# apple/ml-stable-diffusion

Hardware: AMD Instinct MI355X
Metric: diffusion iter/s (UNet steps/s), SD2.1-base 512x512 fp16 (higher is better)
Workload: dtype fp16; 1 GPU; BASELINE config 2: SD2.1-base (865.9 M-parameter UNet), random-init, denoising iteration at 512x512 (64x64 latents), CFG batch 2 per prompt, DDIM, device-resident loop; unet=sd21-base, latent=64, attention=ORIGINAL, prompts_per_gpu=1, global_batch=2, hip_graph=True, parallelism=dp1 (independent prompts per rank, no data-path collective)

## Files before the change

### include/sd_mi355x.h

```cpp
#ifndef SD_MI355X_H
#define SD_MI355X_H

#include <stddef.h>
#include <stdint.h>

#ifdef __cplusplus
extern "C" {
#endif

typedef enum sd_status {
  SD_OK = 0,
  SD_ERR_INVALID_ARGUMENT = -1,
  SD_ERR_NOT_FOUND = -2,
  SD_ERR_HIP = -3,
  SD_ERR_UNSUPPORTED = -4,
  SD_ERR_INTERNAL = -5
} sd_status;

typedef enum sd_dtype { SD_F16 = 0, SD_F32 = 1 } sd_dtype;

typedef enum sd_attention_impl {
  SD_ATTN_ORIGINAL = 0,
  SD_ATTN_SPLIT_EINSUM = 1,
  SD_ATTN_SPLIT_EINSUM_V2 = 2
// ... 103 lines not shown
int sd_text_encoder_encode(sd_text_encoder* t, const int32_t* input_ids, int eos_index, float* last_hidden_state,
                           float* hidden_embeds, float* pooled);

int sd_op_attention(int impl, const void* q, const void* k, const void* v, void* out, int B, int heads, int d,
                    int Sq, int Sk, int variant, int iters, float* ms);
int sd_op_layernorm(const void* x, const float* weight, const float* bias, void* out, int B, int C, int S, float eps,
                    int iters, float* ms);
int sd_op_groupnorm(const void* x, const float* weight, const float* bias, void* out, int B, int C, int H, int W,
                    int groups, float eps, int silu, int iters, float* ms);
int sd_op_groupnorm_shortcut(const void* x0, const void* x1, const float* gn_weight, const float* gn_bias, const void* w, const float* bias,
                             void* out_gn, void* out_sc, int B, int C0, int C1, int H, int W, int N, int groups, float eps, int silu,
                             int side, int iters, float* ms);
int sd_op_conv2d(const void* x, const void* w, const float* bias, const void* res, void* out, int B, int Cin, int H,
                 int W, int Cout, int ksize, int stride, int upsample, int tile, int splitk, int force_generic,
                 int iters, float* ms);
int sd_op_conv2d_groupnorm(const void* x, const void* w, const float* bias, const void* res, const float* gn_weight,
                           const float* gn_bias, void* conv_out, void* out, int B, int Cin, int H, int W, int Cout, int ksize,
                           int groups, float eps, int silu, int tile, int producer_stats, int* entries, int iters, float* ms);
int sd_op_conv2d_groupnorm_proj(const void* x, const void* w, const float* bias, const void* res, const float* gn_weight,
                                const float* gn_bias, const void* proj_w, const float* proj_bias, void* conv_out, void* out, int B,
                                int Cin, int H, int W, int Cout, int ksize, int Nproj, int groups, float eps, int fold, int tile,
                                int* entries, int iters, float* ms);
int sd_op_conv2d_groupnorm_conv3x3(const void* x, const void* w, const float* bias, const void* res, const float* gn_weight,
                                   const float* gn_bias, const void* w2, const float* bias2, const void* res2, void* conv_out, void* out,
                                   int B, int Cin, int H, int W, int Cout, int ksize, int N2, int groups, float eps, int silu, int fold,
                                   int tile, int staging2, int* entries, int iters, float* ms);
int sd_op_ffn_out_proj(const void* g, const void* w1, const float* b1, const void* res1, const void* w2, const float* b2, const void* res2,
                       void* out, float* gn_sums, int B, int C, int S, int groups, int fused, int iters, float* ms);
int sd_op_cross_attention_fused(const void* x, const float* ln_weight, const float* ln_bias, const void* wq, const void* k,
                                const void* v, void* out, int B, int heads, int Sq, int Sk, float eps, int nst, int iters,
// ... 25 lines not shown
```

### ml-stable-diffusion_amd/csrc/capi.cpp

```cpp
#include <cmath>
#include <cstdlib>
#include <cstring>

#include "unet.h"

namespace sd {
extern thread_local std::string g_last_error;
int selftest_mfma();

namespace {

template <typename F>
int guarded(F&& f) {
  try {
    f();
    g_last_error.clear();
    return kOk;
  } catch (const Error& e) {
    g_last_error = e.what();
    return e.code;
  } catch (const std::bad_alloc&) {
    g_last_error = "out of host memory";
    return kInternal;
  } catch (const std::exception& e) {
// ... 452 lines not shown
    const size_t on = (size_t)B * Ho * Wo * Cout;
    half_t* dout = sc.dev<half_t>(on);
    d.out = dout;
    d.B = B; d.Hi = H; d.Wi = W; d.Ho = Ho; d.Wo = Wo;
    d.ksize = ksize; d.stride = stride; d.up = up; d.N = Cout;
    d.tile = tile % 10;
    d.staging = tile / 10;
    if (tile >= 110 && tile <= 116) {
      d.tile = 11;
      d.staging = tile - 110;
    }
    if (tile >= 140 && tile <= 142) {
      d.tile = 12;
      d.staging = tile - 140;
    }
    d.splitk = splitk;
    d.debug = force_generic >= 2 ? force_generic - 1 : 0;
    if (d.debug & 4) d.prof = sc.dev<long long>(8);
    const bool fast = force_generic != 1 && conv_fast_path_ok(d);
    ConvWorkspace ws;
    if (fast && d.tile == 9) {
      SD_REQUIRE(wstream_shape_ok(d), kInvalidArgument, "conv2d: shape not eligible for plan tile 9 (wstream.hip)");
      half_t* wtd = sc.dev<half_t>(wstream_tiled_halves(Cout, Cin, ksize));
      launch_wstream_retile(d.w, wtd, Cout, Cin, ksize, sc.stream);
      d.w_tiled = wtd;
    }
    if (fast && d.tile == 11) {
      SD_REQUIRE(bvgemm_shape_ok(d), kInvalidArgument, "conv2d: shape not eligible for plan tile 11 (bvgemm.hip)");
      half_t* wtd = sc.dev<half_t>(bvgemm_tiled_halves(Cout, Cin));
      launch_bvgemm_retile(d.w, wtd, Cout, Cin, false, sc.stream);
// ... 9 lines not shown
        launch_conv(d, ws, sc.stream);
      else if (small_n)
        launch_conv_small_n(d, nullptr, sc.stream);
      else
        launch_conv_generic(d, 0, sc.stream);
    });
    if (d.prof) {
      long long t[8];
      SD_HIP(hipMemcpy(t, d.prof, sizeof(t), hipMemcpyDeviceToHost));
      fprintf(stderr, "[sd prof] block0: prologue %lld, k-loop %lld, epilogue %lld shader cycles; total %lld cycles = %lld ticks of the 100 MHz wall clock\n",
              t[1] - t[0], t[2] - t[1], t[3] - t[2], t[3] - t[0], t[4]);
    }
    std::vector<half_t> ot(on);
    SD_HIP(hipMemcpy(ot.data(), dout, on * 2, hipMemcpyDeviceToHost));
    nhwc_to_nchw(ot.data(), reinterpret_cast<half_t*>(out), B, Cout, Ho, Wo);
  });
}

int sd_op_conv2d_groupnorm(const void* x, const void* w, const float* bias, const void* res, const float* gn_weight,
                           const float* gn_bias, void* conv_out, void* out, int B, int Cin, int H, int W, int Cout, int ksize,
                           int groups, float eps, int silu, int tile, int producer_stats, int* entries, int iters, float* ms) {
  return guarded([&] {
    SD_REQUIRE(x && w && gn_weight && gn_bias && out, kInvalidArgument, "NULL argument");
    SD_REQUIRE(ksize == 1 || ksize == 3, kInvalidArgument, "conv2d_groupnorm: ksize %d", ksize);
    Scratch sc;
    std::vector<half_t> xt = nchw_to_nhwc(reinterpret_cast<const half_t*>(x), B, Cin, H, W);
    const half_t* wh = reinterpret_cast<const half_t*>(w);
    const int kk = ksize * ksize;
    std::vector<half_t> wt((size_t)Cout * Cin * kk);
    for (int o = 0; o < Cout; ++o)
// ... 5 lines not shown
    d.w = sc.dev<half_t>(wt.size(), wt.data());
    d.bias = bias ? sc.dev<float>(Cout, bias) : nullptr;
    std::vector<half_t> rt;
    if (res) {
      rt = nchw_to_nhwc(reinterpret_cast<const half_t*>(res), B, Cout, H, W);
      d.res = sc.dev<half_t>(rt.size(), rt.data());
    }
    const size_t on = (size_t)B * H * W * Cout;
    half_t* dconv = sc.dev<half_t>(on);
    half_t* dy = sc.dev<half_t>(on);
    d.out = dconv;
    d.B = B; d.Hi = H; d.Wi = W; d.Ho = H; d.Wo = W;
    d.ksize = ksize; d.stride = 1; d.up = 1; d.N = Cout;
    d.tile = tile % 10;
    d.staging = tile / 10;
    d.splitk = 1;
    const bool fast = conv_fast_path_ok(d);
    float* partial = sc.dev<float>(groupnorm_scratch_floats(B, H * W, groups));
    {
      std::vector<float> poison(groupnorm_scratch_floats(B, H * W, groups), 1.0e30f);
      SD_HIP(hipMemcpy(partial, poison.data(), poison.size() * sizeof(float), hipMemcpyHostToDevice));
    }
    if (producer_stats == 1) {
      d.gn_partial = partial;
      d.gn_groups = groups;
    }
    float* dgw = sc.dev<float>(Cout, gn_weight);
    float* dgb = sc.dev<float>(Cout, gn_bias);
    ConvWorkspace ws;
    if (fast && d.tile == 9) {
// ... 937 lines not shown
```

### ml-stable-diffusion_amd/csrc/igemm.hip

```cpp
#include <cstdio>
#include <cstdlib>
#include <cstring>
#include <string>
#include <type_traits>

#include "kernels.h"

namespace sd {

namespace {

constexpr int BK = 64;
constexpr int LDS_ROW = BK + 8;

struct IgemmArgs {
  const half_t* x0;
  const half_t* x1;
  const half_t* w;
  const float* bias;
  const float* temb;
  const half_t* res;
  half_t* out;
  float* partial;
  int C0, C1, Ctot;
// ... 91 lines not shown

__device__ __forceinline__ float xor32_sum(float v) {
  const unsigned u = __float_as_uint(v);
  const auto r = __builtin_amdgcn_permlane32_swap(u, u, false, false);
  const unsigned r0 = r[0], r1 = r[1];
  return __uint_as_float(r0) + __uint_as_float(r1);
}

__device__ __forceinline__ float wave_sum(float v) {
#pragma unroll
  for (int o = 32; o > 0; o >>= 1) v += __shfl_xor(v, o);
  return v;
}
#include "gn_body.inc"

__device__ __forceinline__ void dma16_to_lds(const __amdgpu_buffer_rsrc_t& rs, char* lds, unsigned voffset, int soffset) {
#if defined(__HIP_DEVICE_COMPILE__)
  __builtin_amdgcn_raw_ptr_buffer_load_lds(rs, (__attribute__((address_space(3))) void*)lds, 16, voffset, soffset, 0, 0);
#endif
}

template <int BM, int BN, int WGM, int WGN, int TM, int TN, bool LNF, int NRES = 0>
__device__ __forceinline__ void tile_epilogue(const IgemmArgs& a, floatx16 (&acc)[TM][TN], const float (&ln_a)[TM],
                                              const float (&ln_b)[TM], char* smem, float* sconst, float const_b, float const_t,
                                              float const_c, int m_blk, int n_blk, int wave, int split, bool temb_uniform,
                                              const half8* resv = nullptr, bool use_resv = false) {
  const int tid = threadIdx.x, lane = tid & 63;
  const int wm = wave / WGN, wn = wave % WGN;
  const int frow = lane & 31, hi = lane >> 5;
  if (a.slab) {
#pragma unroll
    for (int i = 0; i < TM; ++i) {
      const int m = m_blk + (wm * TM + i) * 32 + frow;
      if (m >= a.M) continue;
      float* prow = a.partial + ((size_t)split * a.M + m) * a.N;
// ... 579 lines not shown
    tile_epilogue<BM, BN, WGM, WGN, TM, TN, LNF, (RES_PRE ? RIT : 0)>(a, acc, ln_a, ln_b, smem, sconst, const_b, const_t, const_c, m_blk,
                                                                      n_blk, wave, split, temb_uniform, resv, use_resv);
  }
  if (prof) {
    prof_t[3] = clock64();
    a.prof[0] = prof_t[0];
    a.prof[1] = prof_t[1];
    a.prof[2] = prof_t[2];
    a.prof[3] = prof_t[3];
    a.prof[4] = wall_clock64() - prof_w0;
  }
}

constexpr int HALO_W = 18, HALO_ROWS = 180, HALO_PIECES = 23, HALO_LDS_ROWS = 184, HALO_PPW = 6;

template <int N>
__device__ __forceinline__ void wait_vmcnt_barrier() {
  asm volatile("s_waitcnt vmcnt(%0)\n\ts_barrier" ::"n"(N) : "memory");
}
constexpr int halo_mod9(int t) { return ((t % 9) + 9) % 9; }
template <bool GNL = false>
constexpr int halo_x_issued(int tap) {
  const int t = halo_mod9(tap);
  return GNL ? (t == 0 ? 2 : (t <= 4 ? 1 : 0)) : (t < HALO_PPW ? 1 : 0);
}
constexpr size_t halo_lds_bytes(int bn, int d) {
  return ((size_t)2 * HALO_LDS_ROWS * BK + (size_t)d * bn * BK) * sizeof(half_t) + bn * sizeof(float);
}

template <int D, int WR, bool GNL = false>
constexpr int halo_ks_wait_count(int tap) {
  int n = 0;
  for (int i = 2; i <= D - 1; ++i) n += WR + halo_x_issued<GNL>(tap - D + i);
  if (tap == 8 && n > 2 * WR) n = 2 * WR;
// ... 1736 lines not shown
    }
  }
  if (d.tile == 11) {
    SD_REQUIRE(d.w_bv && bvgemm_shape_ok(d), kInvalidArgument, "plan tile 11 (bvgemm.hip) needs the pre-tiled weights and an eligible 1x1 shape");
    launch_bvgemm(d, d.staging, s);
    return 0;
  }
  {
    static const bool sm_on = tune_env_int("SD_SMGEMM", 1) != 0;
    const bool forced = d.tile == 12;
    if (forced || (sm_on && d.tile == 0 && d.splitk == 0 && d.staging == 0 && g_tune.tile == 0 && smgemm_wanted(d))) {
      launch_smgemm(d, forced ? d.staging : 0, s);
      return 0;
    }
  }
  IgemmArgs a = make_args(d);
  Plan p = choose_plan(d, a);
  bool halo = p.tile == 7;
  const bool twins = d.n_twins > 0;
  SD_REQUIRE(!twins || (d.out_mode == kOutHalf && !d.ln_colsum && !d.out_t && !d.debug && reduce_twin_ok(a.HoWo, a.N, d.n_twins, d.twin)),
             kInvalidArgument, "GroupNorm twins need a plain fp16 output and whole (sample, group) slices (HoWo=%d N=%d)", a.HoWo, a.N);
  if (d.gnf_partial && d.ksize == 3) {
    SD_REQUIRE(conv_gn_loader_ok(d) && d.gnf_silu == 1 && d.gnf_gamma && d.gnf_beta && d.gnf_entries >= 1 && d.gnf_entries <= 128 && !twins, kInvalidArgument,
               "GroupNorm in the conv loader: Ctot=%d groups=%d entries=%d up=%d", a.Ctot, d.gnf_groups, d.gnf_entries, d.up);
    p.tile = 7;
    if (p.staging != 2 && p.staging != 3) p.staging = 3;
    p.splitk = 1;
  } else if (d.gnf_partial) {
    SD_REQUIRE(d.ksize == 1 && d.stride == 1 && !d.x1 && d.out_mode == kOutHalf && !d.ln_colsum && !d.out_t && !twins && gemm_pipe_ok(a) &&
                   d.gnf_gamma && d.gnf_beta && d.gnf_groups >= 1 && d.gnf_groups <= 32 && a.K % d.gnf_groups == 0 && a.K <= 2048 &&
// ... 185 lines not shown
```

### ml-stable-diffusion_amd/csrc/kernels.h

```cpp
#pragma once
#include "sd_common.h"

namespace sd {

enum OutMode : int {
  kOutHalf = 0,
  kOutHalfT = 1,
  kOutGeglu = 2,
};

struct GnTwin {
  half_t* y = nullptr;
  int ld = 0, c_off = 0;
  int cpg = 0;
  const float* gamma = nullptr;
  const float* beta = nullptr;
  float eps = 1e-5f;
  int silu = 0;
};

struct ConvDesc {
  const half_t* x0 = nullptr;
  const half_t* x1 = nullptr;
  int C0 = 0, C1 = 0;
// ... 65 lines not shown
bool wsgemm_wanted(const ConvDesc& d);
size_t wsgemm_tiled_halves(int N);
void launch_wsgemm_retile(const half_t* w, half_t* wt, int N, bool geglu, hipStream_t s);
void launch_wsgemm(const ConvDesc& d, hipStream_t s);

bool bvgemm_shape_ok(const ConvDesc& d);
size_t bvgemm_tiled_halves(int N, int K);
void launch_bvgemm_retile(const half_t* w, half_t* wt, int N, int K, bool geglu, hipStream_t s);
void launch_bvgemm(const ConvDesc& d, int variant, hipStream_t s);
bool bvgemm_wanted(const ConvDesc& d);

bool smgemm_shape_ok(const ConvDesc& d, int variant);
bool smgemm_wanted(const ConvDesc& d);
void launch_smgemm(const ConvDesc& d, int variant, hipStream_t s);

void run_calibration(int device, float* out);

int launch_conv_generic(const ConvDesc& d, int act_silu_out, hipStream_t s);

void launch_conv_small_n(const ConvDesc& d, float* out_nchw_f32, hipStream_t s);

enum AttnImpl : int { kAttnOriginal = 0, kAttnSplitEinsum = 1, kAttnSplitEinsumV2 = 2 };

struct AttnDesc {
  const half_t* q = nullptr;
  const half_t* k = nullptr;
  const half_t* vt = nullptr;
  half_t* out = nullptr;
  int B = 1, heads = 1, d = 64, Sq = 0, Sk = 0;
  int ldq = 0, ldk = 0, ldv = 0, ldo = 0;
// ... 165 lines not shown
```

### ml-stable-diffusion_amd/csrc/sd_common.h

```cpp
#pragma once
#include <hip/hip_runtime.h>

#include <cstdint>
#include <cstdio>
#include <cstdlib>
#include <map>
#include <memory>
#include <stdexcept>
#include <string>
#include <atomic>
#include <vector>

namespace sd {

typedef _Float16 half_t;
typedef _Float16 half8 __attribute__((ext_vector_type(8)));
typedef _Float16 half4 __attribute__((ext_vector_type(4)));
typedef _Float16 half2v __attribute__((ext_vector_type(2)));
typedef float floatx16 __attribute__((ext_vector_type(16)));
typedef float floatx4 __attribute__((ext_vector_type(4)));

template <typename V>
__device__ __forceinline__ void out_store(V* p, const V& v) {
#if defined(SD_SC1_STORES) && defined(__HIP_DEVICE_COMPILE__)
  if constexpr (sizeof(V) == 16) {
    typedef unsigned u4_ __attribute__((ext_vector_type(4)));
    asm volatile("global_store_dwordx4 %0, %1, off sc1\n\ts_nop 1" ::"v"(p), "v"(__builtin_bit_cast(u4_, v)) : "memory");
  } else if constexpr (sizeof(V) == 8) {
    typedef unsigned u2_ __attribute__((ext_vector_type(2)));
    asm volatile("global_store_dwordx2 %0, %1, off sc1\n\ts_nop 1" ::"v"(p), "v"(__builtin_bit_cast(u2_, v)) : "memory");
  } else {
    *p = v;
  }
#else
  *p = v;
#endif
}

enum Status : int {
  kOk = 0,
  kInvalidArgument = -1,
  kNotFound = -2,
  kHipError = -3,
  kUnsupported = -4,
  kInternal = -5,
};

struct Error : std::runtime_error {
  int code;
  Error(int c, const std::string& m) : std::runtime_error(m), code(c) {}
};
// ... 75 lines not shown
```

### ml-stable-diffusion_amd/python_hip_stable_diffusion/_lib.py

```python
import ctypes as C
import os

import numpy as np

_HERE = os.path.dirname(os.path.abspath(__file__))
LIB_PATH = os.environ.get("SD_MI355X_LIB", os.path.join(os.path.dirname(_HERE), "lib", "libsdmi355.so"))

SD_MAX_LEVELS = 6
SD_FLAG_DEVICE_PTRS = 1
ATTENTION_IMPLEMENTATIONS = {"ORIGINAL": 0, "SPLIT_EINSUM": 1, "SPLIT_EINSUM_V2": 2}


class LibraryNotBuilt(ImportError):
    pass


class UNetConfig(C.Structure):
    _fields_ = [
        ("batch", C.c_int32), ("in_channels", C.c_int32), ("out_channels", C.c_int32),
        ("height", C.c_int32), ("width", C.c_int32), ("n_levels", C.c_int32),
        ("block_out_channels", C.c_int32 * SD_MAX_LEVELS),
        ("down_cross_attn", C.c_int32 * SD_MAX_LEVELS),
        ("up_cross_attn", C.c_int32 * SD_MAX_LEVELS),
        ("layers_per_block", C.c_int32),
# ... 46 lines not shown
    ("sd_unet_attach_controlnets", _I, [_P, C.POINTER(_P), _I]),
    ("sd_controlnet_set_cond", _I, [_P, _P, _I]),
    ("sd_vae_decoder_create", _I, [C.POINTER(UNetConfig), _P, _I, C.POINTER(_P)]),
    ("sd_vae_decode", _I, [_P, _P, _I, _FP, _I]),
    ("sd_vae_encoder_create", _I, [C.POINTER(UNetConfig), _P, _I, C.POINTER(_P)]),
    ("sd_vae_encode", _I, [_P, _P, _I, _FP, _I]),
    ("sd_text_encoder_create", _I, [_P, _P, _I, C.POINTER(_P)]),
    ("sd_text_encoder_destroy", None, [_P]),
    ("sd_text_encoder_device_bytes", C.c_size_t, [_P]),
    ("sd_text_encoder_encode", _I, [_P, C.POINTER(C.c_int32), _I, _FP, _FP, _FP]),
    ("sd_op_attention", _I, [_I, _P, _P, _P, _P, _I, _I, _I, _I, _I, _I, _I, _FP]),
    ("sd_op_layernorm", _I, [_P, _FP, _FP, _P, _I, _I, _I, _F, _I, _FP]),
    ("sd_op_groupnorm", _I, [_P, _FP, _FP, _P, _I, _I, _I, _I, _I, _F, _I, _I, _FP]),
    ("sd_op_groupnorm_shortcut", _I, [_P, _P, _FP, _FP, _P, _FP, _P, _P, _I, _I, _I, _I, _I, _I, _I, _F, _I, _I, _I, _FP]),
    ("sd_op_conv2d", _I, [_P, _P, _FP, _P, _P, _I, _I, _I, _I, _I, _I, _I, _I, _I, _I, _I, _I, _FP]),
    ("sd_op_conv2d_groupnorm", _I, [_P, _P, _FP, _P, _FP, _FP, _P, _P, _I, _I, _I, _I, _I, _I, _I, _F, _I, _I, _I, C.POINTER(_I), _I, _FP]),
    ("sd_op_conv2d_groupnorm_proj", _I, [_P, _P, _FP, _P, _FP, _FP, _P, _FP, _P, _P, _I, _I, _I, _I, _I, _I, _I, _I, _F, _I, _I, C.POINTER(_I), _I, _FP]),
    ("sd_op_conv2d_groupnorm_conv3x3", _I, [_P, _P, _FP, _P, _FP, _FP, _P, _FP, _P, _P, _P, _I, _I, _I, _I, _I, _I, _I, _I, _F, _I, _I, _I, _I,
                                            C.POINTER(_I), _I, _FP]),
    ("sd_op_cross_attention_fused", _I, [_P, _FP, _FP, _P, _P, _P, _P, _I, _I, _I, _I, _F, _I, _I, _FP]),
    ("sd_op_ffn_out_proj", _I, [_P, _P, _FP, _P, _P, _FP, _P, _P, _FP, _I, _I, _I, _I, _I, _I, _FP]),
    ("sd_op_cross_attention_block", _I, [_P, _FP, _FP, _P, _P, _P, _P, _FP, _P, _P, _FP, _P, _I, _I, _I, _I, _F, _I, _I, _FP]),
    ("sd_op_geglu", _I, [_P, _P, _FP, _P, _I, _I, _I, _I, _FP]),
    ("sd_op_geglu_ln", _I, [_P, _FP, _FP, _P, _FP, _P, _I, _I, _I, C.c_float, _I, _I, _FP]),
    ("sd_op_qkv_ln", _I, [_P, _FP, _FP, _P, _P, _P, _I, _I, _I, C.c_float, C.c_float, _I, _I, _I, _FP]),
    ("sd_op_gn_proj_qkv", _I, [_P, _P, _FP, _FP, _P, _FP, _FP, _FP, _P, _P, _P, _P, _I, _I, _I, _I, _I, C.c_float, C.c_float, C.c_float, _I, _I,
                               C.POINTER(C.c_int), _I, _FP]),
    ("sd_op_timestep_embedding", _I, [_FP, _FP, _I, _I, _I, _F]),
    ("sd_numpy_randn", _I, [C.c_uint32, C.POINTER(C.c_double), C.c_size_t]),
    ("sd_torch_randn", _I, [C.c_uint32, C.POINTER(C.c_double), C.c_size_t]),
# ... 91 lines not shown
    if Cin2 != Cin or k != k2:
        raise ValueError("conv2d: weight shape does not match input")
    up = 2 if upsample else 1
    pad = k // 2
    Ho = (H * up + 2 * pad - k) // stride + 1
    Wo = (W * up + 2 * pad - k) // stride + 1
    bias = None if bias is None else f32(bias)
    res = None if res is None else f16(res)
    out = np.empty((B, Cout, Ho, Wo), np.float16)
    ms = C.c_float(0)
    check(lib().sd_op_conv2d(ptr(x), ptr(w), fptr(bias), ptr(res), ptr(out), B, Cin, H, W, Cout, k, stride,
                             int(upsample), tile, splitk, int(force_generic), iters, C.byref(ms)))
    return out, ms.value


def groupnorm_shortcut(x0, x1, gn_weight, gn_bias, w, bias=None, groups=32, eps=1e-5, silu=True, side=True, iters=1):
    x0, w = f16(x0), f16(w)
    x1 = None if x1 is None else f16(x1)
    B, C0, H, W = x0.shape
    C1 = 0 if x1 is None else x1.shape[1]
    N = w.shape[0]
    w = np.ascontiguousarray(w.reshape(N, -1))
    if w.shape[1] != C0 + C1 or (x1 is not None and x1.shape != (B, C1, H, W)):
        raise ValueError("groupnorm_shortcut: inconsistent shapes")
    gn_weight, gn_bias = f32(gn_weight), f32(gn_bias)
    bias = None if bias is None else f32(bias)
    out_gn = np.empty((B, C0 + C1, H, W), np.float16)
    out_sc = np.empty((B, N, H, W), np.float16)
    ms = C.c_float(0)
    check(lib().sd_op_groupnorm_shortcut(ptr(x0), ptr(x1), fptr(gn_weight), fptr(gn_bias), ptr(w), fptr(bias), ptr(out_gn), ptr(out_sc),
# ... 197 lines not shown
```

Baseline: 236.8 it/s.

## Add conv80 implicit-GEMM 3x3 conv kernel with BN=80 tiles and weight ring

Adds a new 3x3 stride-1 implicit-GEMM conv kernel that uses an 80-wide output-channel tile, a halo-staged activation tile and a D-deep ring of weight stages loaded via buffer-to-LDS DMA. It supports a concatenated second input, upsample-by-2, and bias, temb and residual epilogues. It is auto-selected when the tile count falls between 192 and 256, which aims to fill the CUs better for UNet channel counts such as 320, 640 and 1280 that are multiples of 80. It also adds a conv2d_cat test entry point. The cost is significant new kernel complexity and a risk of mis-selection on some shapes.

```diff
diff --git a/include/sd_mi355x.h b/include/sd_mi355x.h
--- a/include/sd_mi355x.h
+++ b/include/sd_mi355x.h
@@ -141,6 +141,8 @@
 int sd_op_conv2d(const void* x, const void* w, const float* bias, const void* res, void* out, int B, int Cin, int H,
                  int W, int Cout, int ksize, int stride, int upsample, int tile, int splitk, int force_generic,
                  int iters, float* ms);
+int sd_op_conv2d_cat(const void* x0, const void* x1, const void* w, const float* bias, const void* res, void* out, int B, int C0, int C1,
+                     int H, int W, int Cout, int tile, int iters, float* ms);
 int sd_op_conv2d_groupnorm(const void* x, const void* w, const float* bias, const void* res, const float* gn_weight,
                            const float* gn_bias, void* conv_out, void* out, int B, int Cin, int H, int W, int Cout, int ksize,
                            int groups, float eps, int silu, int tile, int producer_stats, int* entries, int iters, float* ms);
diff --git a/ml-stable-diffusion_amd/csrc/capi.cpp b/ml-stable-diffusion_amd/csrc/capi.cpp
--- a/ml-stable-diffusion_amd/csrc/capi.cpp
+++ b/ml-stable-diffusion_amd/csrc/capi.cpp
@@ -490,6 +490,10 @@
       d.tile = 12;
       d.staging = tile - 140;
     }
+    if (tile >= 150 && tile <= 152) {
+      d.tile = 13;
+      d.staging = tile - 150;
+    }
     d.splitk = splitk;
     d.debug = force_generic >= 2 ? force_generic - 1 : 0;
     if (d.debug & 4) d.prof = sc.dev<long long>(8);
@@ -529,6 +533,54 @@
     std::vector<half_t> ot(on);
     SD_HIP(hipMemcpy(ot.data(), dout, on * 2, hipMemcpyDeviceToHost));
     nhwc_to_nchw(ot.data(), reinterpret_cast<half_t*>(out), B, Cout, Ho, Wo);
+  });
+}
+
+int sd_op_conv2d_cat(const void* x0, const void* x1, const void* w, const float* bias, const void* res, void* out, int B, int C0, int C1,
+                     int H, int W, int Cout, int tile, int iters, float* ms) {
+  return guarded([&] {
+    SD_REQUIRE(x0 && x1 && w && out, kInvalidArgument, "NULL argument");
+    SD_REQUIRE(C0 > 0 && C1 > 0, kInvalidArgument, "conv2d_cat: C0 %d C1 %d", C0, C1);
+    Scratch sc;
+    const int Cin = C0 + C1;
+    std::vector<half_t> x0t = nchw_to_nhwc(reinterpret_cast<const half_t*>(x0), B, C0, H, W);
+    std::vector<half_t> x1t = nchw_to_nhwc(reinterpret_cast<const half_t*>(x1), B, C1, H, W);
+    const half_t* wh = reinterpret_cast<const half_t*>(w);
+    std::vector<half_t> wt((size_t)Cout * Cin * 9);
+    for (int o = 0; o < Cout; ++o)
+      for (int c = 0; c < Cin; ++c)
+        for (int t = 0; t < 9; ++t) wt[((size_t)o * 9 + t) * Cin + c] = wh[((size_t)o * Cin + c) * 9 + t];
+    ConvDesc d;
+    d.x0 = sc.dev<half_t>(x0t.size(), x0t.data());
+    d.C0 = C0;
+    d.x1 = sc.dev<half_t>(x1t.size(), x1t.data());
+    d.C1 = C1;
+    d.w = sc.dev<half_t>(wt.size(), wt.data());
+    d.bias = bias ? sc.dev<float>(Cout, bias) : nullptr;
+    std::vector<half_t> rt;
+    if (res) {
+      rt = nchw_to_nhwc(reinterpret_cast<const half_t*>(res), B, Cout, H, W);
+      d.res = sc.dev<half_t>(rt.size(), rt.data());
+    }
+    const size_t on = (size_t)B * H * W * Cout;
+    half_t* dout = sc.dev<half_t>(on);
+    d.out = dout;
+    d.B = B; d.Hi = H; d.Wi = W; d.Ho = H; d.Wo = W;
+    d.ksize = 3; d.stride = 1; d.up = 1; d.N = Cout;
+    d.tile = tile % 10;
+    d.staging = tile / 10;
+    if (tile >= 150 && tile <= 152) {
+      d.tile = 13;
+      d.staging = tile - 150;
+    }
+    SD_REQUIRE(conv_fast_path_ok(d), kInvalidArgument, "conv2d_cat: C0=%d C1=%d N=%d not MFMA-tileable", C0, C1, Cout);
+    ConvWorkspace ws;
+    ws.partial_bytes = conv_workspace_bytes(d);
+    if (ws.partial_bytes) ws.partial = reinterpret_cast<float*>(sc.dev<char>(ws.partial_bytes));
+    sc.timed(iters, ms, [&] { launch_conv(d, ws, sc.stream); });
+    std::vector<half_t> ot(on);
+    SD_HIP(hipMemcpy(ot.data(), dout, on * 2, hipMemcpyDeviceToHost));
+    nhwc_to_nchw(ot.data(), reinterpret_cast<half_t*>(out), B, Cout, H, W);
   });
 }
 
@@ -564,6 +616,10 @@
     d.ksize = ksize; d.stride = 1; d.up = 1; d.N = Cout;
     d.tile = tile % 10;
     d.staging = tile / 10;
+    if (tile >= 150 && tile <= 152) {
+      d.tile = 13;
+      d.staging = tile - 150;
+    }
     d.splitk = 1;
     const bool fast = conv_fast_path_ok(d);
     float* partial = sc.dev<float>(groupnorm_scratch_floats(B, H * W, groups));
diff --git a/ml-stable-diffusion_amd/csrc/conv80.hip b/ml-stable-diffusion_amd/csrc/conv80.hip
--- /dev/null
+++ b/ml-stable-diffusion_amd/csrc/conv80.hip
@@ -0,0 +1,519 @@
+#include <algorithm>
+#include <type_traits>
+
+#include "kernels.h"
+
+namespace sd {
+
+namespace {
+
+constexpr int C8_BK = 64;
+constexpr int C8_BN = 80;
+constexpr int C8_ROWB = 128;
+constexpr int C8_WR = 3;
+constexpr int C8_TN = C8_BN / 16;
+constexpr int C8_WSTAGE = C8_BN * C8_ROWB;
+
+struct C80Args {
+  const half_t* x0;
+  const half_t* x1;
+  const half_t* w;
+  const float* bias;
+  const float* temb;
+  const half_t* res;
+  half_t* out;
+  int C0, C1, Ctot;
+  int B, Hi, Wi, Ho, Wo, up;
+  int N, K;
+  int temb_stride, res_ld;
+  int has_bias, has_temb, has_res;
+  int tiles_x, tiles_y, n_fast;
+  float* gn_partial;
+  int gn_G, gn_cpg;
+};
+
+template <int BM>
+struct C80Geo {
+  static constexpr int TW = BM == 128 ? 16 : 8, TH = 8;
+  static constexpr int HW = TW + 2;
+  static constexpr int HROWS = (TH + 2) * HW;
+  static constexpr int PIECES = (HROWS + 7) / 8;
+  static constexpr int LDS_ROWS = PIECES * 8;
+  static constexpr int PPW = (PIECES + 3) / 4;
+  static constexpr int KY = BM == 128 ? 0 : 4;
+  static constexpr int TMB = BM / 32;
+  static constexpr int KEEP = TMB / 2;
+  static constexpr int HALO_B = LDS_ROWS * C8_ROWB;
+  static_assert(BM == 128 || BM == 64, "tile");
+  static_assert(PPW <= 8, "halo pieces go out in tap steps 0-7");
+};
+
+template <int BM>
+constexpr size_t c80_lds_bytes(int d) {
+  return (size_t)2 * C80Geo<BM>::HALO_B + (size_t)d * C8_WSTAGE + C8_BN * sizeof(float);
+}
+template <int BM>
+constexpr size_t c80_red_bytes() { return (size_t)4 * C80Geo<BM>::KEEP * C8_TN * 64 * 16; }
+constexpr int C8_OROW = C8_BN + 8;
+constexpr int C8_GN_RG = 16;
+
+constexpr int c80_mod9(int t) { return ((t % 9) + 9) % 9; }
+template <int D, int PPW, int MODE>
+constexpr int c80_wait_count(int tap) {
+  int n = 0;
+  for (int u = tap - D + 2; u <= tap - 1; ++u) {
+    if (MODE == 2) n += (u < 0 || u + D < 9) ? C8_WR : 0;
+    else n += C8_WR + ((MODE == 1 ? (u >= 0 && u < PPW) : (c80_mod9(u) < PPW)) ? 1 : 0);
+  }
+  if (MODE != 2 && tap == 8 && n > (8 - PPW) * C8_WR) n = (8 - PPW) * C8_WR;
+  return n;
+}
+template <int D, int PPW, int MODE>
+__device__ __forceinline__ void c80_wait(int tap) {
+  switch (tap) {
+    case 0: wait_vmcnt_barrier<c80_wait_count<D, PPW, MODE>(0)>(); break;
+    case 1: wait_vmcnt_barrier<c80_wait_count<D, PPW, MODE>(1)>(); break;
+    case 2: wait_vmcnt_barrier<c80_wait_count<D, PPW, MODE>(2)>(); break;
+    case 3: wait_vmcnt_barrier<c80_wait_count<D, PPW, MODE>(3)>(); break;
+    case 4: wait_vmcnt_barrier<c80_wait_count<D, PPW, MODE>(4)>(); break;
+    case 5: wait_vmcnt_barrier<c80_wait_count<D, PPW, MODE>(5)>(); break;
+    case 6: wait_vmcnt_barrier<c80_wait_count<D, PPW, MODE>(6)>(); break;
+    case 7: wait_vmcnt_barrier<c80_wait_count<D, PPW, MODE>(7)>(); break;
+    default: wait_vmcnt_barrier<c80_wait_count<D, PPW, MODE>(8)>(); break;
+  }
+}
+
+template <int BM, int D>
+__global__ __launch_bounds__(256, 1) void conv80_kernel(C80Args a) {
+  using G = C80Geo<BM>;
+  constexpr int TW = G::TW, HW = G::HW, PPW = G::PPW, TMB = G::TMB, KEEP = G::KEEP, KY = G::KY;
+  constexpr int ROWB = C8_ROWB, WR = C8_WR, TN = C8_TN, BK = C8_BK;
+  static_assert(D >= 3 && D <= 10, "ring depth: a step's tile is at most one chunk ahead of the chunk after it");
+  static_assert((D - 1) * (WR + 1) <= 63, "vmcnt range");
+  static_assert(c80_lds_bytes<BM>(D) <= 160 * 1024, "LDS");
+  static_assert(c80_red_bytes<BM>() + (size_t)BM * C8_OROW * 2 <= (size_t)2 * G::HALO_B + (size_t)D * C8_WSTAGE, "epilogue buffers fit the K-loop buffers");
+  static_assert((size_t)(C8_GN_RG * 10 * 17 + 2 * C8_BN) * 4 <= c80_red_bytes<BM>(), "statistics scratch fits the exchange buffer");
+  extern __shared__ __attribute__((aligned(16))) char smem[];
+  char* const Xh = smem;
+  char* const Ws = smem + 2 * G::HALO_B;
+  float* const sconst = reinterpret_cast<float*>(Ws + D * C8_WSTAGE);
+
+  const int tid = threadIdx.x, lane = tid & 63;
+  const int wave = __builtin_amdgcn_readfirstlane(tid >> 6);
+  const int wm = wave >> 1, wk = wave & 1;
+  const int g = lane >> 4, r16 = lane & 15;
+  const int H = a.Ho, W = a.Wo;
+  const int ush = a.up >> 1;
+
+  const int n_tiles = a.N / C8_BN;
+  const int m_tiles = a.B * a.tiles_y * a.tiles_x;
+  const int nwg = m_tiles * n_tiles;
+  int bid = blockIdx.x;
+  {
+    int q = nwg >> 3, r = nwg & 7, xcd = bid & 7, idx = bid >> 3;
+    int base = (xcd < r) ? xcd * (q + 1) : r * (q + 1) + (xcd - r) * q;
+    bid = base + idx;
+  }
+  const int bn_idx = a.n_fast ? bid % n_tiles : bid / m_tiles, mt = a.n_fast ? bid / n_tiles : bid % m_tiles;
+  const int b = mt / (a.tiles_y * a.tiles_x);
+  const int trem = mt - b * (a.tiles_y * a.tiles_x);
+  const int ty = trem / a.tiles_x, tx = trem - ty * a.tiles_x;
+  const int y0 = ty * G::TH, x0 = tx * TW;
+  const int n_blk = bn_idx * C8_BN;
+  const int nch = a.Ctot / BK;
+
+  constexpr int VW = KEEP == 2 ? 8 : 4;
+  typedef _Float16 ovec __attribute__((ext_vector_type(VW)));
+  const int opl = wm * (BM / 2) + 16 * (wk * KEEP + (KEEP == 2 ? (g & 1) : 0)) + r16;
+  const int oy = y0 + opl / TW, ox = x0 + opl % TW;
+  const bool o_ok = oy < H && ox < W;
+  const size_t om = (size_t)(b * H + min(oy, H - 1)) * W + min(ox, W - 1);
+  const int ocol = n_blk + (KEEP == 2 ? 8 * (g >> 1) : 4 * g);
+  ovec resv[TN];
+#pragma unroll
+  for (int j = 0; j < TN; ++j) resv[j] = *reinterpret_cast<const ovec*>(a.res + om * a.res_ld + ocol + 16 * j);
+  const int cn = n_blk + min(tid, C8_BN - 1);
+  const float const_b = a.bias[cn], const_t = a.temb[(size_t)b * a.temb_stride + cn];
+  __builtin_amdgcn_sched_barrier(0);
+
+  constexpr unsigned kOob = 0x80000000u;
+  const __amdgpu_buffer_rsrc_t rs_w = __builtin_amdgcn_make_buffer_rsrc(const_cast<half_t*>(a.w), 0, (int)((size_t)a.N * a.K * 2), 0x00020000);
+  const size_t xpix = (size_t)a.B * a.Hi * a.Wi;
+  auto piece_of = [&](int j) { return (wave + 4 * j < G::PIECES) ? wave + 4 * j : G::PIECES - 1; };
+  unsigned hoff0[PPW], hoff1[PPW];
+#pragma unroll
+  for (int j = 0; j < PPW; ++j) {
+    const int hr = 8 * piece_of(j) + (lane >> 3);
+    const int hy = hr / HW, hx = hr - hy * HW;
+    const int iy = y0 - 1 + hy, ix = x0 - 1 + hx;
+    const bool ok = (hr < G::HROWS) && iy >= 0 && iy < H && ix >= 0 && ix < W;
+    const unsigned pix = (unsigned)((b * a.Hi + (iy >> ush)) * a.Wi + (ix >> ush));
+    const unsigned sw = (unsigned)(((lane & 7) ^ (((hx >> 1) + KY * (hy & 1)) & 7)) * 16);
+    hoff0[j] = ok ? pix * (unsigned)a.C0 * 2u + sw : kOob;
+    hoff1[j] = ok ? pix * (unsigned)a.C1 * 2u + sw : kOob;
+  }
+  auto wpiece_of = [&](int i) { return (wave + 4 * i < C8_BN / 8) ? wave + 4 * i : wave + 4 * (i - 1); };
+  unsigned woff[WR];
+#pragma unroll
+  for (int i = 0; i < WR; ++i) {
+    const int r = 8 * wpiece_of(i) + (lane >> 3);
+    woff[i] = (unsigned)(n_blk + r) * (unsigned)a.K * 2u + (unsigned)(((lane & 7) ^ ((r >> 1) & 7)) * 16);
+  }
+#define HALO_SRC(rs, off, soff, ch)                                                                                        \
+  const bool rs##_second = (ch) * BK >= a.C0;                                                           \
+  const __amdgpu_buffer_rsrc_t rs = __builtin_amdgcn_make_buffer_rsrc(                                                     \
+      const_cast<half_t*>(rs##_second ? a.x1 : a.x0), 0, (int)(xpix * (rs##_second ? a.C1 : a.C0) * 2), 0x00020000);       \
+  const int soff = (rs##_second ? (ch) * BK - a.C0 : (ch) * BK) * 2;                                                       \
+  unsigned off[PPW];                                                                                                       \
+  _Pragma("unroll") for (int j_ = 0; j_ < PPW; ++j_) off[j_] = rs##_second ? hoff1[j_] : hoff0[j_];
+  auto issue_x_piece = [&](int j, const __amdgpu_buffer_rsrc_t& rs, unsigned off, int soff, int xstage) {
+    char* dst = Xh + xstage * G::HALO_B + piece_of(j) * 1024;
+    dma16_to_lds(rs, dst, off, soff);
+  };
+  const int total_steps = nch * 9;
+  int iw_koff = 0, iw_tap = 0, iw_slot = 0;
+  auto issue_next_w = [&]() {
+    char* ws = Ws + iw_slot * C8_WSTAGE;
+#pragma unroll
+    for (int i = 0; i < WR; ++i) dma16_to_lds(rs_w, ws + wpiece_of(i) * 1024, woff[i], iw_koff);
+    if (++iw_slot == D) iw_slot = 0;
+    iw_koff += a.Ctot * 2;
+    if (++iw_tap == 9) {
+      iw_tap = 0;
+      iw_koff += (BK - 9 * a.Ctot) * 2;
+    }
+  };
+
+  floatx4 acc[TMB][TN];
+#pragma unroll
+  for (int i = 0; i < TMB; ++i)
+#pragma unroll
+    for (int j = 0; j < TN; ++j) acc[i][j] = floatx4{0.f, 0.f, 0.f, 0.f};
+
+  const int kc = 4 * wk + g;
+  int hrb[TMB];
+  int fpy0 = 0, fpx = 0;
+#pragma unroll
+  for (int i = 0; i < TMB; ++i) {
+    const int ml = wm * (BM / 2) + 16 * i + r16;
+    const int py = ml / TW, px = ml % TW;
+    hrb[i] = (py * HW + px) * ROWB;
+    if (i == 0) { fpy0 = py; fpx = px; }
+  }
+  int xsw[KY ? 2 : 1][3];
+#pragma unroll
+  for (int p = 0; p < (KY ? 2 : 1); ++p)
+#pragma unroll
+    for (int kx = 0; kx < 3; ++kx) xsw[p][kx] = (kc ^ ((((fpx + kx) >> 1) + KY * ((fpy0 + p) & 1)) & 7)) * 16;
+  const int wsw = r16 * ROWB + (kc ^ ((r16 >> 1) & 7)) * 16;
+
+  auto read_step = [&](half8 (&xf)[TMB], half8 (&wf)[TN], const char* xs, const char* ws, int tap) {
+    const int ky = tap / 3, kx = tap - ky * 3;
+    const int toffb = (ky * HW + kx) * ROWB;
+#pragma unroll
+    for (int i = 0; i < TMB; ++i) xf[i] = *reinterpret_cast<const half8*>(xs + hrb[i] + toffb + xsw[KY ? (ky & 1) : 0][kx]);
+#pragma unroll
+    for (int j = 0; j < TN; ++j) wf[j] = *reinterpret_cast<const half8*>(ws + j * 16 * ROWB + wsw);
+  };
+  auto mfma_step = [&](half8 (&xf)[TMB], half8 (&wf)[TN]) {
+#pragma unroll
+    for (int i = 0; i < TMB; ++i)
+#pragma unroll
+      for (int j = 0; j < TN; ++j)
+        acc[i][j] = __builtin_amdgcn_mfma_f32_16x16x32_f16(wf[j], xf[i], acc[i][j], 0, 0, 0);
+  };
+
+  half8 xfA[TMB], wfA[TN], xfB[TMB], wfB[TN];
+  {
+    HALO_SRC(rs0, off0, soff0, 0)
+#pragma unroll
+    for (int j = 0; j < PPW; ++j) issue_x_piece(j, rs0, off0[j], soff0, 0);
+  }
+#pragma unroll
+  for (int p = 0; p < D; ++p) {
+    asm volatile("" ::: "memory");
+    if (p < total_steps) issue_next_w();
+  }
+  if (total_steps >= D) wait_vmcnt_barrier<(D - 1) * WR>();
+  else wait_vmcnt_barrier<0>();
+  read_step(xfA, wfA, Xh, Ws, 0);
+
+  int rd_slot = 0;
+  auto chunk = [&](auto par, auto last, auto first, int ch) {
+    constexpr int PAR = decltype(par)::value;
+    constexpr bool LAST = decltype(last)::value;
+    constexpr int MODE = LAST ? 2 : (decltype(first)::value ? 1 : 0);
+    const int xst = ch & 1;
+    HALO_SRC(rsn, offn, soffn, (LAST ? ch : ch + 1))
+#pragma unroll
+    for (int tap = 0; tap < 9; ++tap) {
+      auto body = [&](half8 (&cx)[TMB], half8 (&cw)[TN], half8 (&nx)[TMB], half8 (&nw)[TN]) {
+        if (LAST && tap == 8) {
+          mfma_step(cx, cw);
+          return;
+        }
+        asm volatile("s_waitcnt lgkmcnt(0)" ::: "memory");
+        c80_wait<D, PPW, MODE>(tap);
+        if (++rd_slot == D) rd_slot = 0;
+        const int tapn = tap == 8 ? 0 : tap + 1;
+        const char* xs = Xh + (tap == 8 ? xst ^ 1 : xst) * G::HALO_B;
+        read_step(nx, nw, xs, Ws + rd_slot * C8_WSTAGE, tapn);
+        if (!LAST || tap + D < 9) issue_next_w();
+        if (!LAST && tap < PPW) issue_x_piece(tap < PPW ? tap : 0, rsn, offn[tap < PPW ? tap : 0], soffn, xst ^ 1);
+        mfma_step(cx, cw);
+        constexpr int NRD = TMB + TN, NMF = TMB * TN;
+        constexpr int RPG = NRD + WR + 1 <= NMF ? 1 : 2;
+        constexpr int RGRP = (NRD + RPG - 1) / RPG;
+#pragma unroll
+        for (int q = 0; q < RGRP; ++q) {
+          __builtin_amdgcn_sched_group_barrier(0x008, 1, 0);
+          __builtin_amdgcn_sched_group_barrier(0x100, RPG, 0);
+        }
+#pragma unroll
+        for (int q = 0; q < WR + 1; ++q) {
+          __builtin_amdgcn_sched_group_barrier(0x008, 1, 0);
+          __builtin_amdgcn_sched_group_barrier(0x010, 1, 0);
+        }
+        __builtin_amdgcn_sched_group_barrier(0x008, NMF - RGRP - WR - 1, 0);
+      };
+      if (((tap + PAR) & 1) == 0) body(xfA, wfA, xfB, wfB);
+      else body(xfB, wfB, xfA, wfA);
+      __builtin_amdgcn_sched_barrier(0);
+    }
+  };
+  {
+    using T = std::true_type;
+    using F = std::false_type;
+    using P0 = std::integral_constant<int, 0>;
+    using P1 = std::integral_constant<int, 1>;
+    if (nch == 1) {
+      chunk(P0{}, T{}, T{}, 0);
+    } else {
+      chunk(P0{}, F{}, T{}, 0);
+      int ch = 1;
+      for (; ch + 2 < nch; ch += 2) {
+        chunk(P1{}, F{}, F{}, ch);
+        chunk(P0{}, F{}, F{}, ch + 1);
+      }
+      if (ch + 2 == nch) {
+        chunk(P1{}, F{}, F{}, ch);
+        chunk(P0{}, T{}, F{}, ch + 1);
+      } else {
+        chunk(P1{}, T{}, F{}, ch);
+      }
+    }
+  }
+  asm volatile("s_waitcnt vmcnt(0) lgkmcnt(0)" ::: "memory");
+  __syncthreads();
+
+  floatx4* const red = reinterpret_cast<floatx4*>(smem);
+#pragma unroll
+  for (int ii = 0; ii < KEEP; ++ii)
+#pragma unroll
+    for (int j = 0; j < TN; ++j) {
+      floatx4 v;
+#pragma unroll
+      for (int e = 0; e < 4; ++e) v[e] = wk ? acc[ii][j][e] : acc[KEEP + ii][j][e];
+      red[((wave * KEEP + ii) * TN + j) * 64 + lane] = v;
+    }
+  if (tid < C8_BN) sconst[tid] = (a.has_bias ? const_b : 0.f) + (a.has_temb ? const_t : 0.f);
+  __syncthreads();
+  floatx4 fin[KEEP][TN];
+#pragma unroll
+  for (int ii = 0; ii < KEEP; ++ii)
+#pragma unroll
+    for (int j = 0; j < TN; ++j) {
+      const floatx4 v = red[(((wave ^ 1) * KEEP + ii) * TN + j) * 64 + lane];
+      const floatx4 bb = *reinterpret_cast<const floatx4*>(sconst + 16 * j + 4 * g);
+#pragma unroll
+      for (int e = 0; e < 4; ++e) fin[ii][j][e] = (wk ? acc[KEEP + ii][j][e] : acc[ii][j][e]) + v[e] + bb[e];
+    }
+  const bool gn = a.gn_partial != nullptr;
+  half_t* const ot = reinterpret_cast<half_t*>(smem + c80_red_bytes<BM>());
+  half_t* const dst = a.out + om * a.N + ocol;
+#pragma unroll
+  for (int j = 0; j < TN; ++j) {
+    ovec o;
+    if constexpr (KEEP == 2) {
+      unsigned lo[2], hi[2];
+#pragma unroll
+      for (int bb = 0; bb < 2; ++bb) {
+        const floatx4 v = fin[bb][j];
+        const half2v h01 = {(half_t)v[0], (half_t)v[1]};
+        const half2v h23 = {(half_t)v[2], (half_t)v[3]};
+        lo[bb] = __builtin_bit_cast(unsigned, h01);
+        hi[bb] = __builtin_bit_cast(unsigned, h23);
+      }
+      const auto s0 = __builtin_amdgcn_permlane16_swap(lo[0], lo[1], false, false);
+      const auto s1 = __builtin_amdgcn_permlane16_swap(hi[0], hi[1], false, false);
+      const unsigned d0 = s0[0], d1 = s1[0], d2 = s0[1], d3 = s1[1];
+      typedef unsigned u4 __attribute__((ext_vector_type(4)));
+      o = __builtin_bit_cast(ovec, (u4){d0, d1, d2, d3});
+    } else {
+      const floatx4 v = fin[0][j];
+      o = __builtin_bit_cast(ovec, half4{(half_t)v[0], (half_t)v[1], (half_t)v[2], (half_t)v[3]});
+    }
+    if (a.has_res) {
+#pragma unroll
+      for (int e = 0; e < VW; ++e) o[e] = (half_t)((float)o[e] + (float)resv[j][e]);
+    }
+    if (o_ok) out_store(reinterpret_cast<ovec*>(dst + 16 * j), o);
+    if (gn) {
+      ovec z;
+#pragma unroll
+      for (int e = 0; e < VW; ++e) z[e] = o_ok ? o[e] : (half_t)0.f;
+      *reinterpret_cast<ovec*>(ot + opl * C8_OROW + (ocol - n_blk) + 16 * j) = z;
+    }
+  }
+  if (!gn) return;
+  __syncthreads();
+  float* const scratch = reinterpret_cast<float*>(smem);
+  float* const chan = scratch + C8_GN_RG * 10 * 17;
+  if (tid < C8_GN_RG * 10) {
+    const int c = tid % 10, rg = tid / 10;
+    float fs[8] = {0.f, 0.f, 0.f, 0.f, 0.f, 0.f, 0.f, 0.f}, fq[8] = {0.f, 0.f, 0.f, 0.f, 0.f, 0.f, 0.f, 0.f};
+#pragma unroll
+    for (int r = 0; r < BM / C8_GN_RG; ++r) {
+      const half8 v = *reinterpret_cast<const half8*>(ot + (rg * (BM / C8_GN_RG) + r) * C8_OROW + 8 * c);
+#pragma unroll
+      for (int e = 0; e < 8; ++e) {
+        const float f = (float)v[e];
+        fs[e] += f;
+        fq[e] = fmaf(f, f, fq[e]);
+      }
+    }
+#pragma unroll
+    for (int e = 0; e < 8; ++e) {
+      scratch[tid * 17 + e] = fs[e];
+      scratch[tid * 17 + 8 + e] = fq[e];
+    }
+  }
+  __syncthreads();
+  if (tid < 2 * C8_BN) {
+    const int which = tid / C8_BN, chn = tid - which * C8_BN;
+    float s = 0.f;
+#pragma unroll
+    for (int rg = 0; rg < C8_GN_RG; ++rg) s += scratch[(rg * 10 + (chn >> 3)) * 17 + which * 8 + (chn & 7)];
+    chan[tid] = s;
+  }
+  __syncthreads();
+  if (tid < C8_BN / a.gn_cpg) {
+    float s = 0.f, q = 0.f;
+    for (int c = tid * a.gn_cpg; c < (tid + 1) * a.gn_cpg; ++c) {
+      s += chan[c];
+      q += chan[C8_BN + c];
+    }
+    float* p = a.gn_partial + (((size_t)b * a.gn_G + n_blk / a.gn_cpg + tid) * kGnMaxSlabs + trem) * 2;
+    p[0] = s;
+    p[1] = q;
+  }
+}
+#undef HALO_SRC
+
+int c80_bm(const ConvDesc& d, int variant) {
+  if (variant == 1) return 128;
+  if (variant == 2) return 64;
+  const long t128 = (long)d.B * cdiv(d.Ho, 8) * cdiv(d.Wo, 16) * (d.N / C8_BN);
+  return t128 >= 192 ? 128 : 64;
+}
+long c80_tiles(const ConvDesc& d, int bm) { return (long)d.B * cdiv(d.Ho, 8) * cdiv(d.Wo, bm == 128 ? 16 : 8) * (d.N / C8_BN); }
+int c80_gn_entries(const ConvDesc& d, int bm) {
+  if (!d.gn_partial || d.gn_groups < 1 || d.N % d.gn_groups != 0) return 0;
+  const int cpg = d.N / d.gn_groups, T = cdiv(d.Ho, 8) * cdiv(d.Wo, bm == 128 ? 16 : 8);
+  return (C8_BN % cpg == 0 && T <= 128) ? T : 0;
+}
+
+template <int BM, int D>
+void launch_c80(const C80Args& a, int nwg, hipStream_t s) {
+  constexpr size_t lds = c80_lds_bytes<BM>(D);
+  auto k = conv80_kernel<BM, D>;
+  static DynLdsOnce once;
+  once.set(k, lds);
+  hipLaunchKernelGGL(k, dim3(nwg), dim3(256), lds, s, a);
+}
+
+}
+
+bool conv80_shape_ok(const ConvDesc& d, int variant) {
+  const int c1 = d.x1 ? d.C1 : 0;
+  if (!(d.ksize == 3 && d.stride == 1 && (d.up == 1 || d.up == 2) && d.pad < 0 && d.out_mode == kOutHalf && !d.ln_colsum && !d.out_t &&
+        !d.gnf_partial && d.n_twins == 0 && !d.debug && variant >= 0 && variant <= 2))
+    return false;
+  if (d.Ho != d.Hi * d.up || d.Wo != d.Wi * d.up || d.Ho < 8 || d.Wo < 8 || d.N < C8_BN) return false;
+  const size_t lim = (size_t)1 << 31;
+  const size_t xpix = (size_t)d.B * d.Hi * d.Wi;
+  return d.N % C8_BN == 0 && d.C0 % C8_BK == 0 && d.C0 >= C8_BK && c1 % C8_BK == 0 && xpix * std::max(d.C0, c1) * 2 < lim &&
+         (size_t)d.N * 9 * (d.C0 + c1) * 2 < lim && c80_tiles(d, c80_bm(d, variant)) <= 65535;
+}
+
+bool conv80_wanted(const ConvDesc& d) {
+  if (!conv80_shape_ok(d, 0)) return false;
+  const int bm = c80_bm(d, 0);
+  const long tiles = c80_tiles(d, bm);
+  if (tiles < 192 || tiles > 256) return false;
+  if (bm == 64 && d.C0 + (d.x1 ? d.C1 : 0) > 640) return false;
+  if (d.gn_partial && c80_gn_entries(d, bm) == 0) return false;
+  return true;
+}
+
+int launch_conv80(const ConvDesc& d, int variant, hipStream_t s) {
+  SD_REQUIRE(conv80_shape_ok(d, variant), kInvalidArgument,
+             "plan tile 13 (conv80.hip): not a 3x3 stride-1 conv it tiles (k=%d stride=%d C0=%d C1=%d N=%d)", d.ksize, d.stride, d.C0,
+             d.x1 ? d.C1 : 0, d.N);
+  const int bm = c80_bm(d, variant);
+  C80Args a;
+  a.x0 = d.x0;
+  a.x1 = d.x1;
+  a.w = d.w;
+  a.C0 = d.C0;
+  a.C1 = d.x1 ? d.C1 : 0;
+  a.Ctot = a.C0 + a.C1;
+  a.B = d.B;
+  a.Hi = d.Hi;
+  a.Wi = d.Wi;
+  a.Ho = d.Ho;
+  a.Wo = d.Wo;
+  a.up = d.up;
+  a.N = d.N;
+  a.K = 9 * a.Ctot;
+  a.bias = d.bias ? d.bias : reinterpret_cast<const float*>(d.w);
+  a.temb = d.temb ? d.temb : reinterpret_cast<const float*>(d.w);
+  a.temb_stride = d.temb ? d.temb_stride : 0;
+  a.res = d.res ? d.res : d.w;
+  a.res_ld = d.res ? d.N : 0;
+  a.has_bias = d.bias != nullptr;
+  a.has_temb = d.temb != nullptr;
+  a.has_res = d.res != nullptr;
+  a.out = d.out;
+  a.tiles_x = cdiv(d.Wo, bm == 128 ? 16 : 8);
+  a.tiles_y = cdiv(d.Ho, 8);
+  const int mt = d.B * a.tiles_x * a.tiles_y, nt = d.N / C8_BN;
+  const double a_bytes = 2.0 * d.B * d.Hi * d.Wi * a.Ctot, w_bytes = 2.0 * a.N * a.K, l2 = 3.5e6;
+  const double m_fast_cost = w_bytes + a_bytes * (a_bytes <= l2 ? std::min(8.0, (double)nt) : (double)nt);
+  const double n_fast_cost = a_bytes + w_bytes * (w_bytes <= l2 ? std::min(8.0, (double)mt) : (double)mt);
+  a.n_fast = nt > 1 && n_fast_cost < m_fast_cost;
+  const int entries = c80_gn_entries(d, bm);
+  a.gn_partial = entries ? d.gn_partial : nullptr;
+  a.gn_G = d.gn_groups;
+  a.gn_cpg = entries ? d.N / d.gn_groups : 1;
+  static const int depth = tune_env_int("SD_CONV80_D", 0);
+  const int D = depth ? depth : 6;
+  static const bool log_plans = tune_env_set("SD_LOG_CONVS");
+  if (log_plans)
+    fprintf(stderr, "[sd conv] k3 s1 up%d C0=%d C1=%d M=%d N=%d K=%d mode=%d tile=13 bm=%d d=%d n_fast=%d\n", a.up, a.C0, a.C1,
+            d.B * d.Ho * d.Wo, a.N, a.K, d.out_mode, bm, D, a.n_fast);
+  const int nwg = mt * nt;
+  if (bm == 128) {
+    if (D <= 6) launch_c80<128, 6>(a, nwg, s);
+    else if (D <= 8) launch_c80<128, 8>(a, nwg, s);
+    else launch_c80<128, 10>(a, nwg, s);
+  } else {
+    if (D <= 6) launch_c80<64, 6>(a, nwg, s);
+    else if (D <= 8) launch_c80<64, 8>(a, nwg, s);
+    else launch_c80<64, 10>(a, nwg, s);
+  }
+  SD_HIP(hipGetLastError());
+  return entries;
+}
+
+}
diff --git a/ml-stable-diffusion_amd/csrc/igemm.hip b/ml-stable-diffusion_amd/csrc/igemm.hip
--- a/ml-stable-diffusion_amd/csrc/igemm.hip
+++ b/ml-stable-diffusion_amd/csrc/igemm.hip
@@ -129,11 +129,6 @@
 }
 #include "gn_body.inc"
 
-__device__ __forceinline__ void dma16_to_lds(const __amdgpu_buffer_rsrc_t& rs, char* lds, unsigned voffset, int soffset) {
-#if defined(__HIP_DEVICE_COMPILE__)
-  __builtin_amdgcn_raw_ptr_buffer_load_lds(rs, (__attribute__((address_space(3))) void*)lds, 16, voffset, soffset, 0, 0);
-#endif
-}
 
 template <int BM, int BN, int WGM, int WGN, int TM, int TN, bool LNF, int NRES = 0>
 __device__ __forceinline__ void tile_epilogue(const IgemmArgs& a, floatx16 (&acc)[TM][TN], const float (&ln_a)[TM],
@@ -743,10 +738,6 @@
 
 constexpr int HALO_W = 18, HALO_ROWS = 180, HALO_PIECES = 23, HALO_LDS_ROWS = 184, HALO_PPW = 6;
 
-template <int N>
-__device__ __forceinline__ void wait_vmcnt_barrier() {
-  asm volatile("s_waitcnt vmcnt(%0)\n\ts_barrier" ::"n"(N) : "memory");
-}
 constexpr int halo_mod9(int t) { return ((t % 9) + 9) % 9; }
 template <bool GNL = false>
 constexpr int halo_x_issued(int tap) {
@@ -2513,6 +2504,12 @@
       return 0;
     }
   }
+  {
+    static const bool c80_on = tune_env_int("SD_CONV80", 1) != 0;
+    const bool forced = d.tile == 13;
+    if (forced || (c80_on && d.tile == 0 && d.splitk == 0 && d.staging == 0 && g_tune.tile == 0 && conv80_wanted(d)))
+      return launch_conv80(d, forced ? d.staging : 0, s);
+  }
   IgemmArgs a = make_args(d);
   Plan p = choose_plan(d, a);
   bool halo = p.tile == 7;
diff --git a/ml-stable-diffusion_amd/csrc/kernels.h b/ml-stable-diffusion_amd/csrc/kernels.h
--- a/ml-stable-diffusion_amd/csrc/kernels.h
+++ b/ml-stable-diffusion_amd/csrc/kernels.h
@@ -103,6 +103,10 @@
 bool smgemm_wanted(const ConvDesc& d);
 void launch_smgemm(const ConvDesc& d, int variant, hipStream_t s);
 
+bool conv80_shape_ok(const ConvDesc& d, int variant);
+bool conv80_wanted(const ConvDesc& d);
+int launch_conv80(const ConvDesc& d, int variant, hipStream_t s);
+
 void run_calibration(int device, float* out);
 
 int launch_conv_generic(const ConvDesc& d, int act_silu_out, hipStream_t s);
diff --git a/ml-stable-diffusion_amd/csrc/sd_common.h b/ml-stable-diffusion_amd/csrc/sd_common.h
--- a/ml-stable-diffusion_amd/csrc/sd_common.h
+++ b/ml-stable-diffusion_amd/csrc/sd_common.h
@@ -35,6 +35,17 @@
 #else
   *p = v;
 #endif
+}
+
+__device__ __forceinline__ void dma16_to_lds(const __amdgpu_buffer_rsrc_t& rs, char* lds, unsigned voffset, int soffset) {
+#if defined(__HIP_DEVICE_COMPILE__)
+  __builtin_amdgcn_raw_ptr_buffer_load_lds(rs, (__attribute__((address_space(3))) void*)lds, 16, voffset, soffset, 0, 0);
+#endif
+}
+
+template <int N>
+__device__ __forceinline__ void wait_vmcnt_barrier() {
+  asm volatile("s_waitcnt vmcnt(%0)\n\ts_barrier" ::"n"(N) : "memory");
 }
 
 enum Status : int {
diff --git a/ml-stable-diffusion_amd/python_hip_stable_diffusion/_lib.py b/ml-stable-diffusion_amd/python_hip_stable_diffusion/_lib.py
--- a/ml-stable-diffusion_amd/python_hip_stable_diffusion/_lib.py
+++ b/ml-stable-diffusion_amd/python_hip_stable_diffusion/_lib.py
@@ -84,6 +84,7 @@
     ("sd_op_groupnorm", _I, [_P, _FP, _FP, _P, _I, _I, _I, _I, _I, _F, _I, _I, _FP]),
     ("sd_op_groupnorm_shortcut", _I, [_P, _P, _FP, _FP, _P, _FP, _P, _P, _I, _I, _I, _I, _I, _I, _I, _F, _I, _I, _I, _FP]),
     ("sd_op_conv2d", _I, [_P, _P, _FP, _P, _P, _I, _I, _I, _I, _I, _I, _I, _I, _I, _I, _I, _I, _FP]),
+    ("sd_op_conv2d_cat", _I, [_P, _P, _P, _FP, _P, _P, _I, _I, _I, _I, _I, _I, _I, _I, _FP]),
     ("sd_op_conv2d_groupnorm", _I, [_P, _P, _FP, _P, _FP, _FP, _P, _P, _I, _I, _I, _I, _I, _I, _I, _F, _I, _I, _I, C.POINTER(_I), _I, _FP]),
     ("sd_op_conv2d_groupnorm_proj", _I, [_P, _P, _FP, _P, _FP, _FP, _P, _FP, _P, _P, _I, _I, _I, _I, _I, _I, _I, _I, _F, _I, _I, C.POINTER(_I), _I, _FP]),
     ("sd_op_conv2d_groupnorm_conv3x3", _I, [_P, _P, _FP, _P, _FP, _FP, _P, _FP, _P, _P, _P, _I, _I, _I, _I, _I, _I, _I, _I, _F, _I, _I, _I, _I,
@@ -205,6 +206,22 @@
     return out, ms.value
 
 
+def conv2d_cat(x0, x1, w, bias=None, res=None, tile=0, iters=1):
+    x0, x1, w = f16(x0), f16(x1), f16(w)
+    B, C0, H, W = x0.shape
+    C1 = x1.shape[1]
+    Cout = w.shape[0]
+    if x1.shape != (B, C1, H, W) or w.shape != (Cout, C0 + C1, 3, 3):
+        raise ValueError("conv2d_cat: inconsistent shapes")
+    bias = None if bias is None else f32(bias)
+    res = None if res is None else f16(res)
+    out = np.empty((B, Cout, H, W), np.float16)
+    ms = C.c_float(0)
+    check(lib().sd_op_conv2d_cat(ptr(x0), ptr(x1), ptr(w), fptr(bias), ptr(res), ptr(out), B, C0, C1, H, W, Cout, tile, iters,
+                                 C.byref(ms)))
+    return out, ms.value
+
+
 def groupnorm_shortcut(x0, x1, gn_weight, gn_bias, w, bias=None, groups=32, eps=1e-5, silu=True, side=True, iters=1):
     x0, w = f16(x0), f16(w)
     x1 = None if x1 is None else f16(x1)
```

Result: faster. 241.5 it/s, median of 6 (+2.0%).
